# Duy1230/Map-Reduced-Approach-for-Vietnamese-Long-Document-Summarization

Hardware: AMD Instinct MI355X
Metric: map-phase chunks/sec (2k-tok chunk, 256-tok summary) at 1/2/4/8 MI355X (higher is better)
Workload: dtype f16

## Files before the change

### include/mapsum.h

```cpp
#ifndef MAPSUM_H
#define MAPSUM_H

#include <stddef.h>
#include <stdint.h>

#ifdef __cplusplus
extern "C" {
#endif

#define MS_ABI_VERSION 3

#define MS_OK 0
#define MS_EIO -5
#define MS_ENOMEM -12
#define MS_EBUSY -16
#define MS_EINVAL -22
#define MS_ENOSPC -28

#define MS_FINISH_EOS 1
#define MS_FINISH_LENGTH 2
#define MS_FINISH_ERROR 3

#define MS_FLAG_IGNORE_EOS 1u

// ... 97 lines not shown
int ms_get_stats(const ms_engine* e, ms_stats* out);
int ms_reset_stats(ms_engine* e);
int ms_set_profiling(ms_engine* e, uint32_t class_mask);
int ms_trace_push(const char* name);
int ms_trace_pop(void);
int ms_synchronize(ms_engine* e);
int ms_set_persist(ms_engine* e, int32_t on);
#define MS_DBG_KPOOL 0
#define MS_DBG_VPOOL 1
#define MS_DBG_DECODE_LOGITS 2
#define MS_DBG_DECODE_X 3
#define MS_DBG_PREFILL_LOGITS 4
int ms_debug_read(ms_engine* e, int32_t which, int64_t offset, void* host, int64_t bytes);
int ms_debug_pk_stamps(uint64_t* out, int32_t n);
int ms_debug_a2_stamps(uint64_t* out, int32_t n);

int ms_forward(ms_engine* e, const int32_t* ids, int32_t n, int32_t n_layers_run,
               float* hidden_out, float* logits_out);
int ms_forward_packed(ms_engine* e, const int32_t* ids, const int32_t* lens, int32_t n_seqs,
                      int32_t n_layers_run, float* hidden_out, float* logits_out);
int ms_submit_forced(ms_engine* e, const int32_t* ids, int32_t n, const int32_t* forced,
                     int32_t n_forced, int32_t num_predict, uint32_t flags, uint64_t tag);

#define MS_EPI_STORE_F16 0
#define MS_EPI_ADD_F32 1
#define MS_EPI_SWIGLU 2
#define MS_EPI_STORE_F32 3
#define MS_EPI_ARGMAX 5
int ms_op_gemm(const void* A, const void* W, void* out, int32_t M, int32_t N, int32_t K,
               int32_t ldo, int32_t epilogue, void* stream);
int ms_op_gemm_resid(const void* A, const void* W, float* x, void* xg_out, const void* gamma, float* ssq_out,
                     int32_t M, int32_t N, int32_t K, void* stream);
int ms_gemm_resid_tiles(int32_t M, int32_t N);
int ms_set_gemm_variant(int32_t variant);
int ms_set_qgemv_gs(int32_t on);
int ms_set_attn_tuning(int32_t combine_grp, int32_t order);
int ms_set_dgemm_kh(int32_t kh);
int ms_set_dgemm_wn(int32_t wn);
int64_t ms_op_gemv_workspace(int32_t M, int32_t N, int32_t K);
int ms_op_gemv(const void* X, const void* W, void* out, int32_t M, int32_t N, int32_t K,
               int32_t ldo, int32_t epilogue, void* workspace, void* stream);
int ms_op_gemv_tuned(const void* X, const void* W, void* out, int32_t M, int32_t N, int32_t K,
                     int32_t ldo, int32_t epilogue, void* workspace, int32_t waves, void* stream);
int ms_op_gemv_strided(const void* X, const void* W, void* out, int32_t M, int32_t N, int32_t K,
                       int32_t ldk, int32_t ldo, int32_t epilogue, void* stream);
int ms_op_gemv_resid(const void* X, const void* W, float* x, void* xg_out, const void* gamma,
                     float* ssq_out, int32_t M, int32_t N, int32_t K, int32_t rt, void* stream);
int ms_op_set_row_scale(const float* ssq, int32_t tiles, int32_t hidden, float eps);
int ms_op_dgemm(const void* X, const void* W, void* out, int32_t M, int32_t N, int32_t K, int32_t S,
// ... 30 lines not shown
```

### map-reduced-approach-for-vietnamese-long-document-summarization_amd/csrc/engine.cpp

```cpp
#include <hip/hip_runtime.h>

#include <algorithm>
#include <cmath>
#include <cstddef>
#include <cstdio>
#include <cstdlib>
#include <cstring>
#include <deque>
#include <array>
#include <functional>
#include <map>
#include <tuple>
#include <memory>
#include <stdexcept>
#include <string>
#include <vector>

#if MS_HAVE_ROCTX
#include <rocprofiler-sdk-roctx/roctx.h>
#else
static inline int roctxRangePushA(const char*) { return 0; }
static inline int roctxRangePop() { return 0; }
#endif

// ... 1909 lines not shown
    REQUIRE(N % 4 == 0 && ((uintptr_t)x & 15) == 0 && ((uintptr_t)xg_out & 7) == 0, MS_EINVAL,
            "gemm_resid: N a multiple of 4, x 16-B and xg 8-B aligned (vector rows)");
    GemmResid gr{(const f16_t*)gamma, (f16_t*)xg_out, ssq_out};
    launch_gemm((const f16_t*)A, (const f16_t*)W, x, M, N, K, N, MS_EPI_ADD_F32, (hipStream_t)stream, nullptr, &gr);
  });
}

int ms_gemm_resid_tiles(int32_t M, int32_t N) { return gemm_resid_tiles(M, N); }

int ms_set_gemm_variant(int32_t v) {
  if (v < 0 || v > 4) return MS_EINVAL;
  set_gemm_variant(v);
  return MS_OK;
}

int ms_set_attn_tuning(int32_t combine_grp, int32_t order) {
  if (combine_grp < 0 || combine_grp > 1 || (order != 0 && order != 3)) return MS_EINVAL;
  set_attn_tuning(combine_grp, order);
  return MS_OK;
}

int ms_set_dgemm_kh(int32_t kh) {
  if (kh != 1 && kh != 2) return MS_EINVAL;
  set_dgemm_kh(kh);
  return MS_OK;
}

int ms_set_dgemm_wn(int32_t wn) {
  if (wn != 4 && wn != 8) return MS_EINVAL;
  set_dgemm_wn(wn);
// ... 33 lines not shown

int ms_op_gemv_strided(const void* X, const void* W, void* out, int32_t M, int32_t N, int32_t K,
                       int32_t ldk, int32_t ldo, int32_t epi, void* stream) {
  return op_guard([&] {
    REQUIRE(X && W && out && N >= 16 && N % 16 == 0 && ldk >= K && ldk % 8 == 0, MS_EINVAL,
            "bad strided gemv operands");
    REQUIRE(epi >= 0 && epi <= 3 && epi != MS_EPI_SWIGLU, MS_EINVAL, "bad epilogue");
    REQUIRE(gemv_supported(M, N, K, epi), MS_EINVAL, "gemv shape unsupported");
    launch_gemv_strided((const f16_t*)X, (const f16_t*)W, out, M, N, K, ldk, ldo, epi, (hipStream_t)stream);
  });
}

int ms_op_gemv_resid(const void* X, const void* W, float* x, void* xg_out, const void* gamma,
                     float* ssq_out, int32_t M, int32_t N, int32_t K, int32_t rt, void* stream) {
  return op_guard([&] {
    REQUIRE(X && W && x && xg_out && gamma && ssq_out && rt >= 1 && rt <= 16 && N % rt == 0, MS_EINVAL,
            "bad gemv_resid operands");
    REQUIRE(gemv_supported(M, N, K, MS_GEMV_EPI_RESID_SSQ), MS_EINVAL, "gemv_resid shape unsupported");
    GemvArgs ga{};
    ga.rt = rt;
    ga.ssq_out = ssq_out;
    ga.gamma = (const f16_t*)gamma;
    ga.xg_out = (f16_t*)xg_out;
    launch_gemv_ex((const f16_t*)X, (const f16_t*)W, x, M, N, K, N, MS_GEMV_EPI_RESID_SSQ, &ga, 0,
                   (hipStream_t)stream);
  });
}

int ms_op_dgemm(const void* X, const void* W, void* out, int32_t M, int32_t N, int32_t K, int32_t S,
                int32_t ldo, int32_t epi, void* stream) {
  return op_guard([&] {
// ... 190 lines not shown
```

### map-reduced-approach-for-vietnamese-long-document-summarization_amd/csrc/gemv_common.h

```cpp
#pragma once
#include "kernels.h"

namespace ms {

__device__ __forceinline__ uint4 ldg16(const void* p) { return *(const uint4*)p; }

__device__ __forceinline__ uint4 ldw16(const void* p) { return *(const uint4*)p; }

__host__ __device__ constexpr int vmcnt_imm(int n) { return (n & 0xF) | ((n >> 4) << 14) | (0x7 << 4) | (0xF << 8); }

__device__ __forceinline__ void lds_sync() {
  __builtin_amdgcn_fence(__ATOMIC_RELEASE, "workgroup", "local");
  __builtin_amdgcn_s_barrier();
  __builtin_amdgcn_fence(__ATOMIC_ACQUIRE, "workgroup", "local");
}

__host__ __device__ inline size_t gemv_x_lds_bytes(int M, int K) {
  return ((size_t)M * K * 2 + 1023) / 1024 * 1024;
}
__device__ __forceinline__ int x_lds(int r, int k, int K) { return r * 2 * K + (((k >> 3) ^ (r & 7)) << 4); }

__device__ __forceinline__ void gemv_dma_x(char* smem, const f16_t* __restrict__ X, int M, int K, int ldx) {
  const int kch = K >> 3, n = M * kch, lane = threadIdx.x & 63, nw = blockDim.x >> 6;
  for (int p = threadIdx.x >> 6; p * 64 < n; p += nw) {
    const int P = min(p * 64 + lane, n - 1);
    const int r = P / kch, c = P - r * kch;
    __builtin_amdgcn_global_load_lds((const void*)(X + (size_t)r * ldx + ((c ^ (r & 7)) << 3)),
                                     (LDS_AS void*)(smem + (size_t)p * 1024), 16, 0, 0);
  }
}

enum { kXGlobal = 0, kXLds = 1, kXRegs = 2 };

constexpr int kRsStage = 4096;
__host__ __device__ inline int rs_stage_floats(const RowScale& rs, int M) {
  const int n = rs.tiles * M;
  return (rs.ssq && n <= kRsStage) ? (n + 63) / 64 * 64 : 0;
}
__host__ __device__ inline size_t gemv_rinv_offset(size_t main_bytes) { return (main_bytes + 15) / 16 * 16; }
__host__ __device__ inline size_t gemv_lds_total(size_t main_bytes, const RowScale& rs, int M) {
  return gemv_rinv_offset(main_bytes) + 64 * 4 + (size_t)rs_stage_floats(rs, M) * 4;
}
template <bool HOLD>
__device__ __forceinline__ float rs_begin(char* smem, size_t rinv_off, const RowScale& rs, int M) {
  const int lane = threadIdx.x & 63, wave = threadIdx.x >> 6, nw = blockDim.x >> 6;
  if constexpr (HOLD)
    if (rs.tiles == 1) return (wave == 0 && lane < M) ? rs.ssq[lane] : 0.f;
// ... 58 lines not shown
}

struct ResidPre {
  float x, g;
};
template <int MT, int NT, int EPI, bool RS>
__device__ __forceinline__ void gemv_epilogue(const float* red, const float* rinv, int M, int N, int ldo,
                                              void* __restrict__ out, int n0, const GemvArgs& ga,
                                              const ResidPre& pre);
__device__ __forceinline__ void gemv_elem(int e, int NT, int n0, int& row, int& col, int& c) {
  const int mn = e >> 8, l = (e >> 2) & 63, j = e & 3;
  row = (mn / NT) * 16 + 4 * (l >> 4) + j;
  c = l & 15;
  col = n0 + (mn % NT) * 16 + c;
}
template <int EPI>
__device__ __forceinline__ ResidPre resid_prefetch(int M, int N, int ldo, const void* out, int n0,
                                                   const GemvArgs& ga) {
  ResidPre p{0.f, 0.f};
  if constexpr (EPI == MS_GEMV_EPI_RESID_SSQ) {
    const int rtv = ga.rt > 0 ? ga.rt : 16;
    if ((int)threadIdx.x < 256) {
      int row, col, c;
      gemv_elem(threadIdx.x, 1, n0, row, col, c);
      if (row < M && c < rtv && col < N) {
        p.x = ((const float*)out)[(size_t)row * ldo + col];
        if (ga.xg_out) p.g = h2f(ga.gamma[col]);
      }
    }
  }
  return p;
}

template <int MT, int NT, int EPI, bool RS = false, bool RS_DONE = false, bool RS_HOLD = true>
__device__ __forceinline__ void gemv_finish(const f32x4 (&acc)[MT][NT], char* smem, size_t rinv_off,
                                            int M, int N, int ldo, void* __restrict__ out, int n0,
                                            const GemvArgs& ga, const ResidPre& pre = ResidPre{0.f, 0.f},
                                            float rs_direct = 0.f) {
  constexpr int ELEMS = MT * NT * 256;
  const int lane = threadIdx.x & 63, wave = threadIdx.x >> 6;
  const float* rinv = (const float*)(smem + rinv_off);
  if constexpr (RS && !RS_DONE) wait_vmcnt0();
  __syncthreads();
  if constexpr (RS && !RS_DONE) rs_finish<RS_HOLD>(smem, rinv_off, ga.rs, M, rs_direct);
  float* red = (float*)smem;
#pragma unroll
  for (int m = 0; m < MT; ++m)
#pragma unroll
    for (int n = 0; n < NT; ++n)
      *(f32x4*)&red[wave * ELEMS + ((m * NT + n) * 64 + lane) * 4] = acc[m][n];
  __syncthreads();
  gemv_epilogue<MT, NT, EPI, RS>(red, rinv, M, N, ldo, out, n0, ga, pre);
}

template <int MT, int NT, int EPI, bool RS>
__device__ __forceinline__ void gemv_epilogue(const float* red, const float* rinv, int M, int N, int ldo,
                                              void* __restrict__ out, int n0, const GemvArgs& ga,
                                              const ResidPre& pre) {
  constexpr int ELEMS = MT * NT * 256;
  const int tid = threadIdx.x;
  const int nthreads = blockDim.x, nw = nthreads >> 6;
  auto rsc = [&](int row) { return RS ? rinv[row] : 1.0f; };
  auto sum_e = [&](int e) {
    float v = 0.f;
    for (int q = 0; q < nw; ++q) v += red[q * ELEMS + e];
// ... 104 lines not shown
```

### map-reduced-approach-for-vietnamese-long-document-summarization_amd/csrc/k_gemv.hip

```cpp
#include "gemv_common.h"

namespace ms {

struct GemvPlan {
  int MT, NT, waves, U, tiles;
};

static GemvPlan gemv_plan(int M, int N, int K, int epi, int force_waves = 0, int rt = 0) {
  GemvPlan p;
  p.MT = (M + 15) / 16;
  p.NT = (epi == MS_GEMV_EPI_SWIGLU) ? 2 : 1;
  const int rows = p.NT == 1 && rt > 0 ? rt : 16 * p.NT;
  p.tiles = (N + rows - 1) / rows;
  const int steps = K / 64;
  int best_w = 0;
  if (force_waves > 0 && steps % force_waves == 0 && steps / force_waves <= 8) {
    best_w = force_waves;
  } else {
    for (int w = 16; w >= 1; --w)
      if (steps % w == 0 && steps / w <= 8) { best_w = w; break; }
  }
  p.waves = best_w;
  p.U = best_w ? steps / best_w : 0;
  return p;
}

size_t gemv_workspace_bytes(int, int, int) { return 256; }

constexpr size_t kMaxLds = 160 * 1024;

static size_t gemv_lds_main(const GemvPlan& p, int M, int K, bool xlds) {
  size_t xs = xlds ? gemv_x_lds_bytes(M, K) : 0;
  const size_t red = (size_t)p.waves * p.MT * p.NT * 256 * 4;
  return xs > red ? xs : red;
}
static size_t gemv_lds_bytes(const GemvPlan& p, int M, int K, bool xlds, const RowScale& rs = RowScale{}) {
  return gemv_lds_total(gemv_lds_main(p, M, K, xlds), rs, M);
}

template <int MT, int NT, int EPI, int U, int XM, bool RS>
__global__ __launch_bounds__(1024) void gemv_kernel(const f16_t* __restrict__ X,
                                                    const f16_t* __restrict__ W,
                                                    void* __restrict__ out, int M, int N, int K,
                                                    int ldk, int ldo, int rinv_off, GemvArgs ga) {
  extern __shared__ __attribute__((aligned(16))) char smem[];
  const int tid = threadIdx.x, lane = tid & 63, wave = tid >> 6;
  const int fr = lane & 15, fg = lane >> 4;
  const int rt = NT == 1 && ga.rt > 0 ? ga.rt : 16;
  const int n0 = blockIdx.x * (NT == 1 ? rt : 16 * NT);
  const int kbeg = wave * U * 64;
  if constexpr (EPI == MS_GEMV_EPI_STORE_F32) {
    X += (size_t)blockIdx.y * K;
// ... 56 lines not shown
      } else {
        const f16_t* xg = X + (size_t)xrow * ldk + kbeg + u * 64 + 16 * fg;
        x0 = as_f16x8(ldg16(xg));
        x1 = as_f16x8(ldg16(xg + 8));
      }
#pragma unroll
      for (int n = 0; n < NT; ++n) {
        acc[m][n] = mfma16(x0, as_f16x8(w[u][n][0]), acc[m][n]);
        acc[m][n] = mfma16(x1, as_f16x8(w[u][n][1]), acc[m][n]);
      }
    }
  }
  gemv_finish<MT, NT, EPI, RS, kRsEarly, false>(acc, smem, rinv_off, M, N, ldo, out, n0, ga, pre);
}

template <int MT, int NT, int EPI, int U, bool RS>
static void gemv_go_rs(const f16_t* X, const f16_t* W, void* out, int M, int N, int K, int ldk,
                       const dim3& grid, const dim3& blk, size_t lds, int ro, int ldo, int xm,
                       const GemvArgs& ga, hipStream_t s) {
  if constexpr (MT * U <= kXRegsMaxFrags) {
    if (xm == kXRegs) {
      MS_LAUNCH((gemv_kernel<MT, NT, EPI, U, kXRegs, RS>), grid, blk, lds, s, X, W, out, M, N, K, ldk,
                ldo, ro, ga);
      return;
    }
  }
  if (xm == kXLds)
    MS_LAUNCH((gemv_kernel<MT, NT, EPI, U, kXLds, RS>), grid, blk, lds, s, X, W, out, M, N, K, ldk,
              ldo, ro, ga);
  else
    MS_LAUNCH((gemv_kernel<MT, NT, EPI, U, kXGlobal, RS>), grid, blk, lds, s, X, W, out, M, N, K, ldk,
              ldo, ro, ga);
}

template <int MT, int NT, int EPI, int U>
static void gemv_go(const f16_t* X, const f16_t* W, void* out, int M, int N, int K, int ldk,
                    int S, int ldo, const GemvPlan& p, size_t lds, int xm, const GemvArgs& ga,
                    hipStream_t s) {
  const dim3 grid(p.tiles, S), blk(64 * p.waves);
  const int ro = (int)gemv_rinv_offset(gemv_lds_main(p, M, K, xm == kXLds));
  if constexpr (EPI == MS_GEMV_EPI_ROPE_KV && MT != 1) {
    return;
  } else if constexpr (gemv_rs_epi<EPI>()) {
    if (ga.rs.ssq) gemv_go_rs<MT, NT, EPI, U, true>(X, W, out, M, N, K, ldk, grid, blk, lds, ro, ldo, xm, ga, s);
    else gemv_go_rs<MT, NT, EPI, U, false>(X, W, out, M, N, K, ldk, grid, blk, lds, ro, ldo, xm, ga, s);
  } else {
    gemv_go_rs<MT, NT, EPI, U, false>(X, W, out, M, N, K, ldk, grid, blk, lds, ro, ldo, xm, ga, s);
  }
}

template <int MT, int NT, int EPI>
static void gemv_go_u(const f16_t* X, const f16_t* W, void* out, int M, int N, int K, int ldk,
                      int S, int ldo, const GemvPlan& p, size_t lds, int xm, const GemvArgs& ga,
                      hipStream_t s) {
#define GU(U_) gemv_go<MT, NT, EPI, U_>(X, W, out, M, N, K, ldk, S, ldo, p, lds, xm, ga, s)
  switch (p.U) {
    case 1: GU(1); break;
    case 2: GU(2); break;
    case 3: GU(3); break;
    case 4: GU(4); break;
    case 5: GU(5); break;
    case 6: GU(6); break;
    case 7: GU(7); break;
    default: GU(8); break;
  }
#undef GU
}

template <int MT>
static void gemv_go_mt(const f16_t* X, const f16_t* W, void* out, int M, int N, int K, int ldk,
                       int S, int ldo, int epi, const GemvPlan& p, size_t lds, int xm,
                       const GemvArgs& ga, hipStream_t s) {
#define GE(NT_, E_) gemv_go_u<MT, NT_, E_>(X, W, out, M, N, K, ldk, S, ldo, p, lds, xm, ga, s)
  switch (epi) {
    case MS_GEMV_EPI_STORE_F16: GE(1, MS_GEMV_EPI_STORE_F16); break;
    case MS_GEMV_EPI_ADD_F32: GE(1, MS_GEMV_EPI_ADD_F32); break;
    case MS_GEMV_EPI_SWIGLU: GE(2, MS_GEMV_EPI_SWIGLU); break;
    case MS_GEMV_EPI_ROPE_KV: GE(1, MS_GEMV_EPI_ROPE_KV); break;
    case MS_GEMV_EPI_ARGMAX: GE(1, MS_GEMV_EPI_ARGMAX); break;
    case MS_GEMV_EPI_RESID_SSQ: GE(1, MS_GEMV_EPI_RESID_SSQ); break;
    default: GE(1, MS_GEMV_EPI_STORE_F32); break;
  }
#undef GE
}

bool gemv_supported(int M, int N, int K, int epi, int rs_tiles) {
  if (M < 1 || M > 64 || K % 64) return false;
  if (epi == MS_GEMV_EPI_ROPE_KV && M > 16) return false;
  if (epi == MS_GEMV_EPI_ARGMAX && N % 16) return false;
  const GemvPlan p = gemv_plan(M, N, K, epi);
  if (p.waves == 0) return false;
  if (epi == MS_GEMV_EPI_RESID_SSQ && p.waves < 4) return false;
  if (epi == MS_GEMV_EPI_ROPE_KV && gemv_lds_bytes(p, M, K, true) > kMaxLds) return false;
  RowScale rs{};
  const bool takes_rs = epi != MS_GEMV_EPI_ARGMAX && epi != MS_GEMV_EPI_ADD_F32 && epi != MS_GEMV_EPI_RESID_SSQ;
  if (rs_tiles > 0 && takes_rs) {
    if (!gemv_rs_supported(M, rs_tiles)) return false;
    rs = make_row_scale(reinterpret_cast<const float*>(16), rs_tiles, 1, 0.f);
  }
  return gemv_lds_bytes(p, M, K, false, rs) <= kMaxLds;
}

static void gemv_dispatch(const f16_t* X, const f16_t* W, void* out, int M, int N, int K, int ldk,
                          int S, int ldo, int epi, const GemvArgs* ga_in, int force_waves,
                          hipStream_t s) {
  if (M <= 0) return;
  const int rt = ga_in ? ga_in->rt : 0;
  const GemvPlan p = gemv_plan(M, N, K, epi, force_waves, rt);
  if (p.waves == 0) return;
  GemvArgs ga{};
  if (ga_in) ga = *ga_in;
  if (epi == MS_GEMV_EPI_ARGMAX || epi == MS_GEMV_EPI_ADD_F32 || epi == MS_GEMV_EPI_RESID_SSQ)
    ga.rs = RowScale{};
  const bool xl = gemv_lds_bytes(p, M, K, true, ga.rs) <= kMaxLds;
  int xm = xl ? kXLds : kXGlobal;
  if (gemv_x_regs_for(epi) && p.MT * p.U <= kXRegsMaxFrags) xm = kXRegs;
  if (ga.rs.ssq && rs_stage_floats(ga.rs, M) == 0) return;
  const size_t lds = gemv_lds_bytes(p, M, K, xm == kXLds, ga.rs);
  if (lds > kMaxLds) return;
  switch (p.MT) {
    case 1: gemv_go_mt<1>(X, W, out, M, N, K, ldk, S, ldo, epi, p, lds, xm, ga, s); break;
    case 2: gemv_go_mt<2>(X, W, out, M, N, K, ldk, S, ldo, epi, p, lds, xm, ga, s); break;
    case 3: gemv_go_mt<3>(X, W, out, M, N, K, ldk, S, ldo, epi, p, lds, xm, ga, s); break;
    default: gemv_go_mt<4>(X, W, out, M, N, K, ldk, S, ldo, epi, p, lds, xm, ga, s); break;
  }
}

void launch_gemv_ex(const f16_t* X, const f16_t* W, void* out, int M, int N, int K, int ldo,
                    int epi, const GemvArgs* ga_in, int force_waves, hipStream_t s) {
  gemv_dispatch(X, W, out, M, N, K, K, 1, ldo, epi, ga_in, force_waves, s);
}

void launch_gemv_strided(const f16_t* X, const f16_t* W, void* out, int M, int N, int K, int ldk,
                         int ldo, int epi, hipStream_t s) {
  gemv_dispatch(X, W, out, M, N, K, ldk, 1, ldo, epi, nullptr, 0, s);
}

bool gemv_rs_supported(int M, int tiles) { return M >= 1 && tiles >= 1 && tiles * M <= kRsStage; }

// ... 49 lines not shown
```

### map-reduced-approach-for-vietnamese-long-document-summarization_amd/csrc/kernels.h

```cpp
#pragma once
#include "common.h"

namespace ms {

struct KVView {
  f16_t* k;
  f16_t* v;
  const int32_t* block_table;
  int32_t max_pages;
  int32_t n_kv_heads;
  int32_t slot_major;
};

constexpr int kPrefillQRows = 128;
struct PrefillAttnArgs {
  const int32_t* seq_qstart;
  const int32_t* seq_qlen;
  const int32_t* seq_kvlen;
  const int32_t* seq_slot;
  const int32_t* qblk;
  int32_t n_qblk;
  const float* cos_tab;
  const float* sin_tab;
};
// ... 107 lines not shown
  f16_t* xg_out;
  RowScale rs;
  int slab_rows;
};
bool gemv_split_supported(int M, int N, int K, int S, int rs_tiles = 0);
bool gemv_rs_supported(int M, int tiles);
void launch_gemv_split(const f16_t* X, const f16_t* W, float* slabs, int M, int N, int K, int S,
                       int force_waves, hipStream_t s, const GemvArgs* ga = nullptr);
void launch_gemv_strided(const f16_t* X, const f16_t* W, void* out, int M, int N, int K, int ldk,
                         int ldo, int epi, hipStream_t s);
void launch_argmax_partials(const void* partials, int rows, int tiles, int32_t* out, hipStream_t s);

bool residual_rmsnorm_supported(int S, int H);
void launch_residual_rmsnorm(float* x, const float* slabs, int S, const f16_t* w, f16_t* y,
                             float* ssq, int rows, int H, hipStream_t s);
size_t gemv_workspace_bytes(int M, int N, int K);
bool gemv_supported(int M, int N, int K, int epi, int rs_tiles = 0);
void launch_gemv(const f16_t* X, const f16_t* W, void* out, int M, int N, int K, int ldo,
                 int epi, void* ws, hipStream_t s);
void launch_gemv_ex(const f16_t* X, const f16_t* W, void* out, int M, int N, int K, int ldo,
                    int epi, const GemvArgs* ga, int force_waves, hipStream_t s);

bool dgemm_supported(int M, int N, int K, int S, int epi, int kh = 0, int wn = 0);
void launch_dgemm(const f16_t* X, const f16_t* W, void* out, int M, int N, int K, int S, int ldo, int epi,
                  hipStream_t s, const RowScale* rs = nullptr, int kh = 0, int wn = 0);
int dgemm_kh_setting();

enum { MS_QT_Q8_0 = 8, MS_QT_Q4_K = 12, MS_QT_Q5_K = 13, MS_QT_Q6_K = 14 };
constexpr int kQ4KBytes = 144, kQ6KBytes = 210, kQ6KPacked = 224;
constexpr int kQ5KBytes = 176;
// ... 126 lines not shown
```

### map-reduced-approach-for-vietnamese-long-document-summarization_amd/mapsum/_lib.py

```python
from __future__ import annotations

import ctypes as C
import os

_HERE = os.path.dirname(os.path.abspath(__file__))
LIB_PATH = os.environ.get("MAPSUM_LIB") or os.path.join(_HERE, "libmapsum.so")

MS_ABI_VERSION = 3
MS_OK, MS_EIO, MS_ENOMEM, MS_EBUSY, MS_EINVAL, MS_ENOSPC = 0, -5, -12, -16, -22, -28
MS_FINISH_EOS, MS_FINISH_LENGTH, MS_FINISH_ERROR = 1, 2, 3
MS_FLAG_IGNORE_EOS = 1
(MS_T_EMBED, MS_T_ATTN_NORM, MS_T_WQ, MS_T_WK, MS_T_WV, MS_T_WO, MS_T_FFN_NORM, MS_T_WGATE,
 MS_T_WUP, MS_T_WDOWN, MS_T_FINAL_NORM, MS_T_LM_HEAD) = range(12)
MS_EPI_STORE_F16, MS_EPI_ADD_F32, MS_EPI_SWIGLU, MS_EPI_STORE_F32 = range(4)
MS_EPI_ARGMAX = 5
GEMM_DEFAULT = 4
MS_GGML_Q8_0, MS_GGML_Q4_K, MS_GGML_Q5_K, MS_GGML_Q6_K = 8, 12, 13, 14
K_GEMM, K_ATTN_PREFILL, K_GEMV, K_ATTN_DECODE, K_LMHEAD, K_MISC, K_PERSIST = range(7)
MS_DBG_KPOOL, MS_DBG_VPOOL, MS_DBG_DECODE_LOGITS, MS_DBG_DECODE_X, MS_DBG_PREFILL_LOGITS = range(5)
MS_SAMPLE_MAX_TOPK, MS_SAMPLE_MAX_WINDOW = 256, 256

EXPORTED = (
    "ms_create", "ms_destroy", "ms_last_error", "ms_load_weight", "ms_init_synthetic",
    "ms_load_weight_q", "ms_init_synthetic_q", "ms_init_synthetic_q8_0", "ms_init_synthetic_q5_k_m", "ms_op_dequant", "ms_op_quant_rows", "ms_op_qgemv", "ms_op_qgemv_split", "ms_op_qgemv_resid", "ms_op_qdgemm",
    "ms_submit", "ms_step", "ms_poll", "ms_pending", "ms_get_stats", "ms_reset_stats",
    "ms_set_profiling", "ms_synchronize", "ms_forward", "ms_op_gemm", "ms_op_gemv_workspace",
    "ms_op_gemv", "ms_op_gemv_tuned", "ms_op_gemv_split", "ms_op_dgemm", "ms_op_residual_rmsnorm", "ms_op_rmsnorm",
    "ms_op_argmax", "ms_op_argmax_partials", "ms_set_gemm_variant", "ms_set_qgemv_gs", "ms_set_attn_tuning", "ms_set_dgemm_kh", "ms_set_dgemm_wn",
    "ms_weight_regions", "ms_quant_manifest", "ms_declare_weight_q",
    "ms_forward_packed", "ms_submit_forced", "ms_set_eos_ids", "ms_op_gemv_strided",
    "ms_op_gemv_resid", "ms_op_set_row_scale", "ms_op_gemm_resid", "ms_gemm_resid_tiles",
    "ms_trace_push", "ms_trace_pop", "ms_debug_a2_stamps", "ms_set_persist", "ms_debug_read", "ms_debug_pk_stamps",
    "ms_submit_sampled", "ms_op_sample",
)


class MsConfig(C.Structure):
    _fields_ = [("abi_version", C.c_int32),
                ("n_layers", C.c_int32), ("hidden", C.c_int32), ("n_heads", C.c_int32),
                ("n_kv_heads", C.c_int32), ("head_dim", C.c_int32), ("ffn", C.c_int32),
                ("vocab", C.c_int32),
                ("rope_theta", C.c_float), ("rope_factor", C.c_float),
                ("rope_low_freq_factor", C.c_float), ("rope_high_freq_factor", C.c_float),
                ("rope_orig_ctx", C.c_int32), ("norm_eps", C.c_float), ("tie_embeddings", C.c_int32),
                ("device", C.c_int32), ("max_batch", C.c_int32), ("max_ctx", C.c_int32),
                ("max_prefill_tokens", C.c_int32), ("n_pages", C.c_int32), ("n_eos", C.c_int32),
                ("eos_ids", C.c_int32 * 8)]

# ... 68 lines not shown
        "ms_op_gemv_resid": (i32, [vp, vp, vp, vp, vp, vp, i32, i32, i32, i32, vp]),
        "ms_op_qgemv_resid": (i32, [vp, i32, vp, vp, vp, vp, vp, i32, i32, i32, i32, vp]),
        "ms_op_set_row_scale": (i32, [vp, i32, i32, C.c_float]),
        "ms_op_gemm_resid": (i32, [vp, vp, vp, vp, vp, vp, i32, i32, i32, vp]),
        "ms_gemm_resid_tiles": (i32, [i32, i32]),
        "ms_submit_forced": (i32, [vp, pi32, i32, pi32, i32, i32, u32, u64]),
        "ms_op_gemm": (i32, [vp, vp, vp, i32, i32, i32, i32, i32, vp]),
        "ms_op_gemv_workspace": (i64, [i32, i32, i32]),
        "ms_op_gemv": (i32, [vp, vp, vp, i32, i32, i32, i32, i32, vp, vp]),
        "ms_op_gemv_tuned": (i32, [vp, vp, vp, i32, i32, i32, i32, i32, vp, i32, vp]),
        "ms_op_gemv_split": (i32, [vp, vp, vp, i32, i32, i32, i32, i32, vp]),
        "ms_op_dgemm": (i32, [vp, vp, vp, i32, i32, i32, i32, i32, i32, vp]),
        "ms_op_residual_rmsnorm": (i32, [vp, vp, i32, vp, vp, vp, i32, i32, vp]),
        "ms_op_rmsnorm": (i32, [vp, vp, vp, vp, i32, i32, vp, vp]),
        "ms_set_gemm_variant": (i32, [i32]),
        "ms_set_qgemv_gs": (i32, [i32]),
        "ms_set_attn_tuning": (i32, [i32, i32]),
        "ms_set_dgemm_kh": (i32, [i32]),
        "ms_set_dgemm_wn": (i32, [i32]),
        "ms_op_argmax": (i32, [vp, i32, i32, vp, vp]),
        "ms_op_argmax_partials": (i32, [vp, i32, i32, vp, vp]),
        "ms_weight_regions": (i32, [vp, C.POINTER(vp), C.POINTER(i64), i32]),
        "ms_quant_manifest": (i32, [vp, pi32, i32]),
        "ms_declare_weight_q": (i32, [vp, i32, i32, i32]),
        "ms_trace_push": (i32, [C.c_char_p]),
        "ms_trace_pop": (i32, []),
        "ms_set_persist": (i32, [vp, i32]),
        "ms_debug_read": (i32, [vp, i32, i64, vp, i64]),
        "ms_debug_pk_stamps": (i32, [vp, i32]),
        "ms_debug_a2_stamps": (i32, [vp, i32]),
    }
    for name, (res, args) in sig.items():
        if ab and not hasattr(lib, name):
            continue
        fn = getattr(lib, name)
        fn.restype = res
        fn.argtypes = args
    return lib


def check(rc: int, handle=None, what: str = "") -> int:
    if rc < 0:
        msg = load().ms_last_error(handle)
        raise RuntimeError(f"libmapsum {what} failed ({rc}): {msg.decode() if msg else ''}")
    return rc
# ... 23 lines not shown
```

Measured before the change: 12.87.

## Add weight-first GEMV load ordering and per-wave swizzled X LDS slices

```diff
diff --git a/include/mapsum.h b/include/mapsum.h
--- a/include/mapsum.h
+++ b/include/mapsum.h
@@ -135,6 +135,7 @@
 int ms_debug_read(ms_engine* e, int32_t which, int64_t offset, void* host, int64_t bytes);
 int ms_debug_pk_stamps(uint64_t* out, int32_t n);
 int ms_debug_a2_stamps(uint64_t* out, int32_t n);
+int ms_debug_gemv_stamps(uint64_t* out, int32_t n);
 
 int ms_forward(ms_engine* e, const int32_t* ids, int32_t n, int32_t n_layers_run,
                float* hidden_out, float* logits_out);
@@ -154,6 +155,8 @@
                      int32_t M, int32_t N, int32_t K, void* stream);
 int ms_gemm_resid_tiles(int32_t M, int32_t N);
 int ms_set_gemm_variant(int32_t variant);
+#define MS_GEMV_ORDER_DEFAULT (-1)
+int ms_set_gemv_order(int32_t order);
 int ms_set_qgemv_gs(int32_t on);
 int ms_set_attn_tuning(int32_t combine_grp, int32_t order);
 int ms_set_dgemm_kh(int32_t kh);
diff --git a/map-reduced-approach-for-vietnamese-long-document-summarization_amd/csrc/engine.cpp b/map-reduced-approach-for-vietnamese-long-document-summarization_amd/csrc/engine.cpp
--- a/map-reduced-approach-for-vietnamese-long-document-summarization_amd/csrc/engine.cpp
+++ b/map-reduced-approach-for-vietnamese-long-document-summarization_amd/csrc/engine.cpp
@@ -1947,6 +1947,18 @@
   return MS_OK;
 }
 
+int ms_set_gemv_order(int32_t order) {
+  if (order < -1 || order > 2) return MS_EINVAL;
+  set_gemv_order(order);
+  return MS_OK;
+}
+
+int ms_debug_gemv_stamps(uint64_t* out, int32_t n) {
+  if (!out || n < 0) return MS_EINVAL;
+  ms::gemv_stamps(reinterpret_cast<unsigned long long*>(out), n);
+  return MS_OK;
+}
+
 int ms_set_attn_tuning(int32_t combine_grp, int32_t order) {
   if (combine_grp < 0 || combine_grp > 1 || (order != 0 && order != 3)) return MS_EINVAL;
   set_attn_tuning(combine_grp, order);
@@ -2010,7 +2022,7 @@
 int ms_op_gemv_resid(const void* X, const void* W, float* x, void* xg_out, const void* gamma,
                      float* ssq_out, int32_t M, int32_t N, int32_t K, int32_t rt, void* stream) {
   return op_guard([&] {
-    REQUIRE(X && W && x && xg_out && gamma && ssq_out && rt >= 1 && rt <= 16 && N % rt == 0, MS_EINVAL,
+    REQUIRE(X && W && x && xg_out && gamma && ssq_out && rt >= 1 && rt <= 16 && N >= 1, MS_EINVAL,
             "bad gemv_resid operands");
     REQUIRE(gemv_supported(M, N, K, MS_GEMV_EPI_RESID_SSQ), MS_EINVAL, "gemv_resid shape unsupported");
     GemvArgs ga{};
diff --git a/map-reduced-approach-for-vietnamese-long-document-summarization_amd/csrc/gemv_common.h b/map-reduced-approach-for-vietnamese-long-document-summarization_amd/csrc/gemv_common.h
--- a/map-reduced-approach-for-vietnamese-long-document-summarization_amd/csrc/gemv_common.h
+++ b/map-reduced-approach-for-vietnamese-long-document-summarization_amd/csrc/gemv_common.h
@@ -30,7 +30,31 @@
   }
 }
 
-enum { kXGlobal = 0, kXLds = 1, kXRegs = 2 };
+__host__ __device__ inline size_t gemv_xw_lds_bytes(int M, int K) { return (size_t)((M + 7) >> 3) * K * 16; }
+__device__ __forceinline__ int xw_swz(int r) {
+  const int t = r >> 1;
+  return ((((t >> 1) ^ (t >> 2)) & 1) << 2) | ((t & 1) << 1) | ((t >> 2) & 1);
+}
+__device__ __forceinline__ int xw_lds(int r, int u, int c, int mp) {
+  return (u * mp * 8 + r) * 128 + ((c ^ xw_swz(r)) << 4);
+}
+template <int U>
+__device__ __forceinline__ void gemv_dma_x_wave(char* smem, const f16_t* __restrict__ X, int M, int ldx,
+                                                int kbeg) {
+  const int lane = threadIdx.x & 63, wave = threadIdx.x >> 6, mp = (M + 7) >> 3;
+  char* base = smem + (size_t)wave * U * mp * 1024;
+#pragma unroll 1
+  for (int j = 0; j < mp; ++j) {
+    const int r = j * 8 + (lane >> 3);
+    const f16_t* src = X + (size_t)min(r, M - 1) * ldx + kbeg + (((lane & 7) ^ xw_swz(r)) << 3);
+#pragma unroll
+    for (int u = 0; u < U; ++u)
+      __builtin_amdgcn_global_load_lds((const void*)(src + u * 64), (LDS_AS void*)(base + (size_t)(u * mp + j) * 1024),
+                                       16, 0, 0);
+  }
+}
+
+enum { kXGlobal = 0, kXLds = 1, kXRegs = 2, kXWave = 3 };
 
 constexpr int kRsStage = 4096;
 __host__ __device__ inline int rs_stage_floats(const RowScale& rs, int M) {
@@ -119,7 +143,7 @@
   c = l & 15;
   col = n0 + (mn % NT) * 16 + c;
 }
-template <int EPI>
+template <int EPI, bool RAW = false>
 __device__ __forceinline__ ResidPre resid_prefetch(int M, int N, int ldo, const void* out, int n0,
                                                    const GemvArgs& ga) {
   ResidPre p{0.f, 0.f};
@@ -130,18 +154,22 @@
       gemv_elem(threadIdx.x, 1, n0, row, col, c);
       if (row < M && c < rtv && col < N) {
         p.x = ((const float*)out)[(size_t)row * ldo + col];
-        if (ga.xg_out) p.g = h2f(ga.gamma[col]);
+        if (ga.xg_out) p.g = RAW ? __uint_as_float((unsigned)ga.gamma[col]) : h2f(ga.gamma[col]);
       }
     }
   }
   return p;
+}
+__device__ __forceinline__ void resid_gain(ResidPre& p) {
+  asm volatile("" : "+v"(p.g));
+  p.g = h2f((f16_t)__float_as_uint(p.g));
 }
 
 template <int MT, int NT, int EPI, bool RS = false, bool RS_DONE = false, bool RS_HOLD = true>
 __device__ __forceinline__ void gemv_finish(const f32x4 (&acc)[MT][NT], char* smem, size_t rinv_off,
                                             int M, int N, int ldo, void* __restrict__ out, int n0,
                                             const GemvArgs& ga, const ResidPre& pre = ResidPre{0.f, 0.f},
-                                            float rs_direct = 0.f) {
+                                            float rs_direct = 0.f, unsigned long long* t_red = nullptr) {
   constexpr int ELEMS = MT * NT * 256;
   const int lane = threadIdx.x & 63, wave = threadIdx.x >> 6;
   const float* rinv = (const float*)(smem + rinv_off);
@@ -154,6 +182,7 @@
 #pragma unroll
     for (int n = 0; n < NT; ++n)
       *(f32x4*)&red[wave * ELEMS + ((m * NT + n) * 64 + lane) * 4] = acc[m][n];
+  if (t_red) *t_red = __builtin_amdgcn_s_memrealtime();
   __syncthreads();
   gemv_epilogue<MT, NT, EPI, RS>(red, rinv, M, N, ldo, out, n0, ga, pre);
 }
diff --git a/map-reduced-approach-for-vietnamese-long-document-summarization_amd/csrc/k_gemv.hip b/map-reduced-approach-for-vietnamese-long-document-summarization_amd/csrc/k_gemv.hip
--- a/map-reduced-approach-for-vietnamese-long-document-summarization_amd/csrc/k_gemv.hip
+++ b/map-reduced-approach-for-vietnamese-long-document-summarization_amd/csrc/k_gemv.hip
@@ -29,13 +29,175 @@
 
 constexpr size_t kMaxLds = 160 * 1024;
 
-static size_t gemv_lds_main(const GemvPlan& p, int M, int K, bool xlds) {
-  size_t xs = xlds ? gemv_x_lds_bytes(M, K) : 0;
+static size_t gemv_lds_main(const GemvPlan& p, int M, int K, int xm) {
+  size_t xs = xm == kXLds ? gemv_x_lds_bytes(M, K) : xm == kXWave ? gemv_xw_lds_bytes(M, K) : 0;
   const size_t red = (size_t)p.waves * p.MT * p.NT * 256 * 4;
   return xs > red ? xs : red;
 }
-static size_t gemv_lds_bytes(const GemvPlan& p, int M, int K, bool xlds, const RowScale& rs = RowScale{}) {
-  return gemv_lds_total(gemv_lds_main(p, M, K, xlds), rs, M);
+static size_t gemv_lds_bytes(const GemvPlan& p, int M, int K, int xm, const RowScale& rs = RowScale{}) {
+  return gemv_lds_total(gemv_lds_main(p, M, K, xm), rs, M);
+}
+
+constexpr int kGvStampBlocks = 1024, kGvStamps = 32;
+__device__ unsigned long long g_gemv_stamps[kGvStampBlocks * kGvStamps];
+#define GV_STAMP(k)                                     \
+  do {                                                  \
+    if constexpr (STAMP) {                              \
+      __builtin_amdgcn_sched_barrier(0);                \
+      ts[k] = __builtin_amdgcn_s_memrealtime();         \
+      __builtin_amdgcn_sched_barrier(0);                \
+    }                                                   \
+  } while (0)
+
+template <int MT, int NT, int EPI, int U, int XM, bool RS, bool WF, bool STAMP>
+__device__ __forceinline__ void gemv_body(const f16_t* __restrict__ X, const f16_t* __restrict__ W,
+                                          void* __restrict__ out, int M, int N, int K, int ldk, int ldo,
+                                          int rinv_off, const GemvArgs& ga) {
+  static_assert(!WF || XM == kXLds || XM == kXWave, "weight-first applies to the DMA-staged forms");
+  static_assert(XM != kXWave || WF, "per-wave slices come with the weight-first order");
+  extern __shared__ __attribute__((aligned(16))) char smem[];
+  const int tid = threadIdx.x, lane = tid & 63, wave = tid >> 6;
+  const int fr = lane & 15, fg = lane >> 4;
+  unsigned long long ts[STAMP ? 12 : 1] = {};
+  GV_STAMP(0);
+  const int rt = NT == 1 && ga.rt > 0 ? ga.rt : 16;
+  const int n0 = blockIdx.x * (NT == 1 ? rt : 16 * NT);
+  const int kbeg = wave * U * 64;
+  if constexpr (EPI == MS_GEMV_EPI_STORE_F32) {
+    X += (size_t)blockIdx.y * K;
+    W += (size_t)blockIdx.y * K;
+    out = (float*)out + (size_t)blockIdx.y * (ga.slab_rows > 0 ? ga.slab_rows : M) * ldo;
+  }
+  constexpr bool kXL = XM == kXLds || XM == kXWave;
+  constexpr bool kRsEarly = kXL && NT == 1;
+  constexpr bool kBar = XM == kXLds || (RS && NT == 1);
+  constexpr int kAfterX = WF ? (U - 1) * NT * 2 : U * NT * 2;
+
+  uint4 w[U][NT][2];
+  if constexpr (WF) {
+#pragma unroll
+    for (int n = 0; n < NT; ++n) {
+      const int wrow = NT == 1 ? n0 + min(fr, rt - 1) : n0 + n * 16 + fr;
+      const f16_t* wp = W + (size_t)min(wrow, N - 1) * ldk + kbeg + 16 * fg;
+      w[0][n][0] = ldw16(wp);
+      w[0][n][1] = ldw16(wp + 8);
+    }
+    GV_STAMP(2);
+    __builtin_amdgcn_sched_barrier(0);
+  }
+  if constexpr (RS) rs_begin<false>(smem, rinv_off, ga.rs, M);
+  ResidPre pre = resid_prefetch<EPI, WF>(M, N, ldo, out, n0, ga);
+  if constexpr (XM == kXLds) gemv_dma_x(smem, X, M, K, ldk);
+  if constexpr (XM == kXWave) gemv_dma_x_wave<U>(smem, X, M, ldk, kbeg);
+  uint4 xr[XM == kXRegs ? U : 1][XM == kXRegs ? MT : 1][2];
+  if constexpr (XM == kXRegs) {
+#pragma unroll
+    for (int u = 0; u < U; ++u)
+#pragma unroll
+      for (int m = 0; m < MT; ++m) {
+        const f16_t* xg = X + (size_t)min(m * 16 + fr, M - 1) * ldk + kbeg + u * 64 + 16 * fg;
+        xr[u][m][0] = ldg16(xg);
+        xr[u][m][1] = ldg16(xg + 8);
+      }
+  }
+  GV_STAMP(3);
+  __builtin_amdgcn_sched_barrier(0);
+  if constexpr (WF) {
+#pragma unroll
+    for (int u = 1; u < U; ++u)
+#pragma unroll
+      for (int n = 0; n < NT; ++n) {
+        const int wrow = NT == 1 ? n0 + min(fr, rt - 1) : n0 + n * 16 + fr;
+        const f16_t* wp = W + (size_t)min(wrow, N - 1) * ldk + kbeg + 16 * fg;
+        w[u][n][0] = ldw16(wp + u * 64);
+        w[u][n][1] = ldw16(wp + u * 64 + 8);
+      }
+  } else {
+#pragma unroll
+    for (int n = 0; n < NT; ++n) {
+      const int wrow = NT == 1 ? n0 + min(fr, rt - 1) : n0 + n * 16 + fr;
+      const f16_t* wp = W + (size_t)min(wrow, N - 1) * ldk + kbeg + 16 * fg;
+#pragma unroll
+      for (int u = 0; u < U; ++u) {
+        w[u][n][0] = ldw16(wp + u * 64);
+        w[u][n][1] = ldw16(wp + u * 64 + 8);
+        if (n == 0 && u == 0) GV_STAMP(2);
+      }
+    }
+  }
+  GV_STAMP(4);
+  if constexpr (kXL) {
+    __builtin_amdgcn_sched_barrier(0);
+    __builtin_amdgcn_s_waitcnt(vmcnt_imm(kAfterX));
+    GV_STAMP(5);
+    if constexpr (kBar) __builtin_amdgcn_s_barrier();
+    GV_STAMP(6);
+    if constexpr (RS && NT == 1) rs_finish<false>(smem, rinv_off, ga.rs, M, 0.f);
+  }
+
+  f32x4 acc[MT][NT];
+#pragma unroll
+  for (int m = 0; m < MT; ++m)
+#pragma unroll
+    for (int n = 0; n < NT; ++n) acc[m][n] = f32x4{0.f, 0.f, 0.f, 0.f};
+  const int mp = (M + 7) >> 3;
+  const char* xw = smem + (size_t)wave * U * mp * 1024;
+#pragma unroll
+  for (int u = 0; u < U; ++u) {
+    if constexpr (STAMP) {
+      if (u == 0) {
+        __builtin_amdgcn_s_waitcnt(vmcnt_imm(WF ? (U - 1) * NT * 2 : (U - 1) * 2));
+        GV_STAMP(7);
+      }
+      if (u == U - 1) {
+        __builtin_amdgcn_s_waitcnt(vmcnt_imm(0));
+        GV_STAMP(8);
+      }
+    }
+#pragma unroll
+    for (int m = 0; m < MT; ++m) {
+      const int xrow = min(m * 16 + fr, M - 1);
+      f16x8 x0, x1;
+      if constexpr (XM == kXRegs) {
+        x0 = as_f16x8(xr[u][m][0]);
+        x1 = as_f16x8(xr[u][m][1]);
+      } else if constexpr (XM == kXLds) {
+        const int k0 = kbeg + u * 64 + 16 * fg;
+        x0 = *(const f16x8*)(smem + x_lds(xrow, k0, K));
+        x1 = *(const f16x8*)(smem + x_lds(xrow, k0 + 8, K));
+      } else if constexpr (XM == kXWave) {
+        x0 = *(const f16x8*)(xw + xw_lds(xrow, u, 2 * fg, mp));
+        x1 = *(const f16x8*)(xw + xw_lds(xrow, u, 2 * fg + 1, mp));
+      } else {
+        const f16_t* xg = X + (size_t)xrow * ldk + kbeg + u * 64 + 16 * fg;
+        x0 = as_f16x8(ldg16(xg));
+        x1 = as_f16x8(ldg16(xg + 8));
+      }
+#pragma unroll
+      for (int n = 0; n < NT; ++n) {
+        acc[m][n] = mfma16(x0, as_f16x8(w[u][n][0]), acc[m][n]);
+        acc[m][n] = mfma16(x1, as_f16x8(w[u][n][1]), acc[m][n]);
+      }
+    }
+  }
+  if constexpr (WF && EPI == MS_GEMV_EPI_RESID_SSQ) resid_gain(pre);
+  GV_STAMP(9);
+  unsigned long long* t_red = nullptr;
+  if constexpr (STAMP) t_red = &ts[10];
+  gemv_finish<MT, NT, EPI, RS, kRsEarly, false>(acc, smem, rinv_off, M, N, ldo, out, n0, ga, pre, 0.f, t_red);
+  if constexpr (STAMP) {
+    GV_STAMP(11);
+    const int nw = blockDim.x >> 6, blk = blockIdx.y * gridDim.x + blockIdx.x;
+    if (lane == 0 && (wave == 0 || wave == nw - 1) && blk < kGvStampBlocks) {
+      unsigned hw, xcc;
+      asm volatile("s_getreg_b32 %0, hwreg(HW_REG_HW_ID)" : "=s"(hw));
+      asm volatile("s_getreg_b32 %0, hwreg(HW_REG_XCC_ID)" : "=s"(xcc));
+      ts[1] = ((unsigned long long)xcc << 32) | hw;
+      unsigned long long* dst = g_gemv_stamps + (size_t)blk * kGvStamps + (wave == 0 ? 0 : 16);
+#pragma unroll
+      for (int k = 0; k < 12; ++k) dst[k] = ts[k];
+    }
+  }
 }
 
 template <int MT, int NT, int EPI, int U, int XM, bool RS>
@@ -122,46 +284,104 @@
   gemv_finish<MT, NT, EPI, RS, kRsEarly, false>(acc, smem, rinv_off, M, N, ldo, out, n0, ga, pre);
 }
 
+template <int MT, int NT, int EPI, int U, int XM, bool RS>
+__global__ __launch_bounds__(1024) void gemv_wf_kernel(const f16_t* __restrict__ X,
+                                                       const f16_t* __restrict__ W,
+                                                       void* __restrict__ out, int M, int N, int K,
+                                                       int ldk, int ldo, int rinv_off, GemvArgs ga) {
+  gemv_body<MT, NT, EPI, U, XM, RS, true, false>(X, W, out, M, N, K, ldk, ldo, rinv_off, ga);
+}
+
+template <int NT, int EPI, int U, int XM, bool RS, bool WF>
+__global__ __launch_bounds__(1024) void gemv_stamp_kernel(const f16_t* __restrict__ X,
+                                                          const f16_t* __restrict__ W,
+                                                          void* __restrict__ out, int M, int N, int K,
+                                                          int ldk, int ldo, int rinv_off, GemvArgs ga) {
+  gemv_body<1, NT, EPI, U, XM, RS, WF, true>(X, W, out, M, N, K, ldk, ldo, rinv_off, ga);
+}
+
+void gemv_stamps(unsigned long long* host, int n) {
+  n = std::min(n, kGvStampBlocks * kGvStamps);
+  (void)hipMemcpyFromSymbol(host, HIP_SYMBOL(g_gemv_stamps), (size_t)n * sizeof(unsigned long long));
+  void* p = nullptr;
+  if (hipGetSymbolAddress(&p, HIP_SYMBOL(g_gemv_stamps)) == hipSuccess)
+    (void)hipMemset(p, 0, sizeof(unsigned long long) * kGvStampBlocks * kGvStamps);
+}
+
+static bool gemv_stamps_on() {
+  static const bool on = [] { const char* e = getenv("MS_GEMV_STAMPS"); return e && atoi(e); }();
+  return on;
+}
+
+enum { kGcQkv = 0, kGcO, kGcGateUp, kGcDown, kGcLmHead, kGcCount };
+static int g_gemv_class_order[kGcCount] = {0, 2, 1, 2, 0};
+static int g_gemv_order = [] {
+  const char* e = getenv("MS_GEMV_ORDER");
+  if (!e || !e[0]) return -1;
+  auto dig = [](char c) { return c >= '0' && c <= '2' ? c - '0' : 0; };
+  if (!e[1]) return dig(e[0]);
+  for (int i = 0; i < kGcCount && e[i]; ++i) g_gemv_class_order[i] = dig(e[i]);
+  return -1;
+}();
+void set_gemv_order(int v) { g_gemv_order = v; }
+static int gemv_order_for(int epi, int N, int U) {
+  if (g_gemv_order >= 0) return g_gemv_order;
+  if (epi == MS_GEMV_EPI_SWIGLU) return g_gemv_class_order[kGcGateUp];
+  if (epi == MS_GEMV_EPI_RESID_SSQ) return g_gemv_class_order[U <= 4 ? kGcO : kGcDown];
+  if (epi == MS_GEMV_EPI_ARGMAX || (epi == MS_GEMV_EPI_STORE_F32 && N >= 65536)) return g_gemv_class_order[kGcLmHead];
+  if (epi == MS_GEMV_EPI_STORE_F32) return g_gemv_class_order[kGcQkv];
+  return 0;
+}
+
 template <int MT, int NT, int EPI, int U, bool RS>
 static void gemv_go_rs(const f16_t* X, const f16_t* W, void* out, int M, int N, int K, int ldk,
-                       const dim3& grid, const dim3& blk, size_t lds, int ro, int ldo, int xm,
+                       const dim3& grid, const dim3& blk, size_t lds, int ro, int ldo, int xm, int ord,
                        const GemvArgs& ga, hipStream_t s) {
+#define GL(...) MS_LAUNCH((__VA_ARGS__), grid, blk, lds, s, X, W, out, M, N, K, ldk, ldo, ro, ga)
   if constexpr (MT * U <= kXRegsMaxFrags) {
     if (xm == kXRegs) {
-      MS_LAUNCH((gemv_kernel<MT, NT, EPI, U, kXRegs, RS>), grid, blk, lds, s, X, W, out, M, N, K, ldk,
-                ldo, ro, ga);
+      GL(gemv_kernel<MT, NT, EPI, U, kXRegs, RS>);
       return;
     }
   }
-  if (xm == kXLds)
-    MS_LAUNCH((gemv_kernel<MT, NT, EPI, U, kXLds, RS>), grid, blk, lds, s, X, W, out, M, N, K, ldk,
-              ldo, ro, ga);
-  else
-    MS_LAUNCH((gemv_kernel<MT, NT, EPI, U, kXGlobal, RS>), grid, blk, lds, s, X, W, out, M, N, K, ldk,
-              ldo, ro, ga);
+  constexpr bool kStampEpi = EPI == MS_GEMV_EPI_STORE_F32 || EPI == MS_GEMV_EPI_SWIGLU ||
+                             EPI == MS_GEMV_EPI_RESID_SSQ || EPI == MS_GEMV_EPI_ARGMAX;
+  if constexpr (MT == 1 && (U == 1 || U == 3 || U == 8) && kStampEpi) {
+    if (gemv_stamps_on() && (xm == kXLds || xm == kXWave)) {
+      if (xm == kXWave) GL(gemv_stamp_kernel<NT, EPI, U, kXWave, RS, true>);
+      else if (ord) GL(gemv_stamp_kernel<NT, EPI, U, kXLds, RS, true>);
+      else GL(gemv_stamp_kernel<NT, EPI, U, kXLds, RS, false>);
+      return;
+    }
+  }
+  if (xm == kXWave) GL(gemv_wf_kernel<MT, NT, EPI, U, kXWave, RS>);
+  else if (xm == kXLds && ord) GL(gemv_wf_kernel<MT, NT, EPI, U, kXLds, RS>);
+  else if (xm == kXLds) GL(gemv_kernel<MT, NT, EPI, U, kXLds, RS>);
+  else GL(gemv_kernel<MT, NT, EPI, U, kXGlobal, RS>);
+#undef GL
 }
 
 template <int MT, int NT, int EPI, int U>
 static void gemv_go(const f16_t* X, const f16_t* W, void* out, int M, int N, int K, int ldk,
-                    int S, int ldo, const GemvPlan& p, size_t lds, int xm, const GemvArgs& ga,
+                    int S, int ldo, const GemvPlan& p, size_t lds, int xm, int ord, const GemvArgs& ga,
                     hipStream_t s) {
   const dim3 grid(p.tiles, S), blk(64 * p.waves);
-  const int ro = (int)gemv_rinv_offset(gemv_lds_main(p, M, K, xm == kXLds));
+  const int ro = (int)gemv_rinv_offset(gemv_lds_main(p, M, K, xm));
   if constexpr (EPI == MS_GEMV_EPI_ROPE_KV && MT != 1) {
     return;
   } else if constexpr (gemv_rs_epi<EPI>()) {
-    if (ga.rs.ssq) gemv_go_rs<MT, NT, EPI, U, true>(X, W, out, M, N, K, ldk, grid, blk, lds, ro, ldo, xm, ga, s);
-    else gemv_go_rs<MT, NT, EPI, U, false>(X, W, out, M, N, K, ldk, grid, blk, lds, ro, ldo, xm, ga, s);
+    if (ga.rs.ssq) gemv_go_rs<MT, NT, EPI, U, true>(X, W, out, M, N, K, ldk, grid, blk, lds, ro, ldo, xm, ord, ga, s);
+    else gemv_go_rs<MT, NT, EPI, U, false>(X, W, out, M, N, K, ldk, grid, blk, lds, ro, ldo, xm, ord, ga, s);
   } else {
-    gemv_go_rs<MT, NT, EPI, U, false>(X, W, out, M, N, K, ldk, grid, blk, lds, ro, ldo, xm, ga, s);
+    gemv_go_rs<MT, NT, EPI, U, false>(X, W, out, M, N, K, ldk, grid, blk, lds, ro, ldo, xm, ord, ga, s);
   }
 }
 
 template <int MT, int NT, int EPI>
 static void gemv_go_u(const f16_t* X, const f16_t* W, void* out, int M, int N, int K, int ldk,
-                      int S, int ldo, const GemvPlan& p, size_t lds, int xm, const GemvArgs& ga,
+                      int S, int ldo, const GemvPlan& p, size_t lds, int xm, int ord, const GemvArgs& ga,
                       hipStream_t s) {
-#define GU(U_) gemv_go<MT, NT, EPI, U_>(X, W, out, M, N, K, ldk, S, ldo, p, lds, xm, ga, s)
+#define GU(U_) gemv_go<MT, NT, EPI, U_>(X, W, out, M, N, K, ldk, S, ldo, p, lds, xm, ord, ga, s)
   switch (p.U) {
     case 1: GU(1); break;
     case 2: GU(2); break;
@@ -177,9 +397,9 @@
 
 template <int MT>
 static void gemv_go_mt(const f16_t* X, const f16_t* W, void* out, int M, int N, int K, int ldk,
-                       int S, int ldo, int epi, const GemvPlan& p, size_t lds, int xm,
+                       int S, int ldo, int epi, const GemvPlan& p, size_t lds, int xm, int ord,
                        const GemvArgs& ga, hipStream_t s) {
-#define GE(NT_, E_) gemv_go_u<MT, NT_, E_>(X, W, out, M, N, K, ldk, S, ldo, p, lds, xm, ga, s)
+#define GE(NT_, E_) gemv_go_u<MT, NT_, E_>(X, W, out, M, N, K, ldk, S, ldo, p, lds, xm, ord, ga, s)
   switch (epi) {
     case MS_GEMV_EPI_STORE_F16: GE(1, MS_GEMV_EPI_STORE_F16); break;
     case MS_GEMV_EPI_ADD_F32: GE(1, MS_GEMV_EPI_ADD_F32); break;
@@ -199,14 +419,14 @@
   const GemvPlan p = gemv_plan(M, N, K, epi);
   if (p.waves == 0) return false;
   if (epi == MS_GEMV_EPI_RESID_SSQ && p.waves < 4) return false;
-  if (epi == MS_GEMV_EPI_ROPE_KV && gemv_lds_bytes(p, M, K, true) > kMaxLds) return false;
+  if (epi == MS_GEMV_EPI_ROPE_KV && gemv_lds_bytes(p, M, K, kXLds) > kMaxLds) return false;
   RowScale rs{};
   const bool takes_rs = epi != MS_GEMV_EPI_ARGMAX && epi != MS_GEMV_EPI_ADD_F32 && epi != MS_GEMV_EPI_RESID_SSQ;
   if (rs_tiles > 0 && takes_rs) {
     if (!gemv_rs_supported(M, rs_tiles)) return false;
     rs = make_row_scale(reinterpret_cast<const float*>(16), rs_tiles, 1, 0.f);
   }
-  return gemv_lds_bytes(p, M, K, false, rs) <= kMaxLds;
+  return gemv_lds_bytes(p, M, K, kXGlobal, rs) <= kMaxLds;
 }
 
 static void gemv_dispatch(const f16_t* X, const f16_t* W, void* out, int M, int N, int K, int ldk,
@@ -220,17 +440,19 @@
   if (ga_in) ga = *ga_in;
   if (epi == MS_GEMV_EPI_ARGMAX || epi == MS_GEMV_EPI_ADD_F32 || epi == MS_GEMV_EPI_RESID_SSQ)
     ga.rs = RowScale{};
-  const bool xl = gemv_lds_bytes(p, M, K, true, ga.rs) <= kMaxLds;
+  const bool xl = gemv_lds_bytes(p, M, K, kXLds, ga.rs) <= kMaxLds;
   int xm = xl ? kXLds : kXGlobal;
+  const int ord = xl ? gemv_order_for(epi, N, p.U) : 0;
+  if (ord == 2 && gemv_lds_bytes(p, M, K, kXWave, ga.rs) <= kMaxLds) xm = kXWave;
   if (gemv_x_regs_for(epi) && p.MT * p.U <= kXRegsMaxFrags) xm = kXRegs;
   if (ga.rs.ssq && rs_stage_floats(ga.rs, M) == 0) return;
-  const size_t lds = gemv_lds_bytes(p, M, K, xm == kXLds, ga.rs);
+  const size_t lds = gemv_lds_bytes(p, M, K, xm, ga.rs);
   if (lds > kMaxLds) return;
   switch (p.MT) {
-    case 1: gemv_go_mt<1>(X, W, out, M, N, K, ldk, S, ldo, epi, p, lds, xm, ga, s); break;
-    case 2: gemv_go_mt<2>(X, W, out, M, N, K, ldk, S, ldo, epi, p, lds, xm, ga, s); break;
-    case 3: gemv_go_mt<3>(X, W, out, M, N, K, ldk, S, ldo, epi, p, lds, xm, ga, s); break;
-    default: gemv_go_mt<4>(X, W, out, M, N, K, ldk, S, ldo, epi, p, lds, xm, ga, s); break;
+    case 1: gemv_go_mt<1>(X, W, out, M, N, K, ldk, S, ldo, epi, p, lds, xm, ord, ga, s); break;
+    case 2: gemv_go_mt<2>(X, W, out, M, N, K, ldk, S, ldo, epi, p, lds, xm, ord, ga, s); break;
+    case 3: gemv_go_mt<3>(X, W, out, M, N, K, ldk, S, ldo, epi, p, lds, xm, ord, ga, s); break;
+    default: gemv_go_mt<4>(X, W, out, M, N, K, ldk, S, ldo, epi, p, lds, xm, ord, ga, s); break;
   }
 }
 
diff --git a/map-reduced-approach-for-vietnamese-long-document-summarization_amd/csrc/kernels.h b/map-reduced-approach-for-vietnamese-long-document-summarization_amd/csrc/kernels.h
--- a/map-reduced-approach-for-vietnamese-long-document-summarization_amd/csrc/kernels.h
+++ b/map-reduced-approach-for-vietnamese-long-document-summarization_amd/csrc/kernels.h
@@ -145,6 +145,8 @@
 bool residual_rmsnorm_supported(int S, int H);
 void launch_residual_rmsnorm(float* x, const float* slabs, int S, const f16_t* w, f16_t* y,
                              float* ssq, int rows, int H, hipStream_t s);
+void set_gemv_order(int v);
+void gemv_stamps(unsigned long long* host, int n);
 size_t gemv_workspace_bytes(int M, int N, int K);
 bool gemv_supported(int M, int N, int K, int epi, int rs_tiles = 0);
 void launch_gemv(const f16_t* X, const f16_t* W, void* out, int M, int N, int K, int ldo,
diff --git a/map-reduced-approach-for-vietnamese-long-document-summarization_amd/mapsum/_lib.py b/map-reduced-approach-for-vietnamese-long-document-summarization_amd/mapsum/_lib.py
--- a/map-reduced-approach-for-vietnamese-long-document-summarization_amd/mapsum/_lib.py
+++ b/map-reduced-approach-for-vietnamese-long-document-summarization_amd/mapsum/_lib.py
@@ -15,6 +15,7 @@
 MS_EPI_STORE_F16, MS_EPI_ADD_F32, MS_EPI_SWIGLU, MS_EPI_STORE_F32 = range(4)
 MS_EPI_ARGMAX = 5
 GEMM_DEFAULT = 4
+GEMV_ORDER_DEFAULT = -1
 MS_GGML_Q8_0, MS_GGML_Q4_K, MS_GGML_Q5_K, MS_GGML_Q6_K = 8, 12, 13, 14
 K_GEMM, K_ATTN_PREFILL, K_GEMV, K_ATTN_DECODE, K_LMHEAD, K_MISC, K_PERSIST = range(7)
 MS_DBG_KPOOL, MS_DBG_VPOOL, MS_DBG_DECODE_LOGITS, MS_DBG_DECODE_X, MS_DBG_PREFILL_LOGITS = range(5)
@@ -31,7 +32,7 @@
     "ms_forward_packed", "ms_submit_forced", "ms_set_eos_ids", "ms_op_gemv_strided",
     "ms_op_gemv_resid", "ms_op_set_row_scale", "ms_op_gemm_resid", "ms_gemm_resid_tiles",
     "ms_trace_push", "ms_trace_pop", "ms_debug_a2_stamps", "ms_set_persist", "ms_debug_read", "ms_debug_pk_stamps",
-    "ms_submit_sampled", "ms_op_sample",
+    "ms_submit_sampled", "ms_op_sample", "ms_set_gemv_order", "ms_debug_gemv_stamps",
 )
 
 
@@ -130,6 +131,7 @@
         "ms_op_residual_rmsnorm": (i32, [vp, vp, i32, vp, vp, vp, i32, i32, vp]),
         "ms_op_rmsnorm": (i32, [vp, vp, vp, vp, i32, i32, vp, vp]),
         "ms_set_gemm_variant": (i32, [i32]),
+        "ms_set_gemv_order": (i32, [i32]),
         "ms_set_qgemv_gs": (i32, [i32]),
         "ms_set_attn_tuning": (i32, [i32, i32]),
         "ms_set_dgemm_kh": (i32, [i32]),
@@ -145,6 +147,7 @@
         "ms_debug_read": (i32, [vp, i32, i64, vp, i64]),
         "ms_debug_pk_stamps": (i32, [vp, i32]),
         "ms_debug_a2_stamps": (i32, [vp, i32]),
+        "ms_debug_gemv_stamps": (i32, [vp, i32]),
     }
     for name, (res, args) in sig.items():
         if ab and not hasattr(lib, name):
```

Result: faster. 13.08, median of 6 (+1.6%).
